# jtdingx/quadrupedal_loco

Measured on AMD Instinct MI355X. Metric: MPC QP solves/sec (Go1 SRBD N=10, 12 forces); p99 solve us, higher is better.
Workload: dtype f32

## Files before the change

### include/qloco.h

```cpp
#ifndef QLOCO_H
#define QLOCO_H

#include <stddef.h>
#include <stdint.h>

#ifdef __cplusplus
extern "C" {
#endif

#define QLOCO_ABI_VERSION 1

typedef enum qloco_status {
  QLOCO_OK = 0,
  QLOCO_MAX_ITER = 1,
  QLOCO_INFEASIBLE = 2,
  QLOCO_NAN = 3,
  QLOCO_BAD_SIZE = 4,
  QLOCO_NOT_PD = 5,
  QLOCO_DEGENERATE = 6,
  QLOCO_UB_PATH = 7,
  QLOCO_SOLVED_INACCURATE = 8,
  QLOCO_ERR_ARG = 100,
  QLOCO_ERR_DEVICE = 101,
  QLOCO_ERR_NO_GPU = 102
} qloco_status;

const char *qloco_status_string(int status);
int qloco_abi_version(void);
const char *qloco_last_error(void);

typedef struct qloco_srbd_spec {
  int32_t horizon;
  int32_t feet_per_step;
  int32_t contacts_per_step;
  int32_t output_frame;
  float dt;
  float mass;
  float inertia[9];
  float q_weights[13];
  float r_weights[12];
  float mu;
  float fz_min, fz_max;
  float rho, sigma, alpha, eps_abs, eps_rel;
  int32_t max_iter, check_termination, scaling, adaptive_rho, adaptive_rho_interval;
  float adaptive_rho_tolerance;
  int32_t warm_start;
  int32_t polish;
  int32_t literal_full_qp;
  int32_t reserved[5];
} qloco_srbd_spec;

#define QLOCO_SRBD_PERSIST_LEN(N) (100 * (N) + 4)

void qloco_srbd_spec_default(qloco_srbd_spec *spec);

int qloco_srbd_lit_tables(const qloco_srbd_spec *spec, float *gtab, int64_t gtab_len,
                          float *s_scale, float *gmx, int32_t *served);

int qloco_srbd_max_stance_vars(void);

int qloco_srbd_solve(const qloco_srbd_spec *spec, int64_t batch, const float *x0,
                     const float *x_ref, const float *feet, const uint8_t *contacts,
                     float *u0, float *u, int32_t *status, int32_t *iters, float *obj,
                     float *warm, void *stream);

int qloco_srbd_solve_ex(const qloco_srbd_spec *spec, int64_t batch, const float *x0,
                        const float *x_ref, const float *feet, const uint8_t *contacts,
                        float *u0, float *u, int32_t *status, int32_t *iters,
                        int32_t *rho_updates, float *obj, float *warm,
                        int32_t max_stance_legs, void *stream);

int64_t qloco_srbd_place_bytes(int64_t batch);
int qloco_srbd_solve_placed(const qloco_srbd_spec *spec, int64_t batch, const float *x0,
                            const float *x_ref, const float *feet, const uint8_t *contacts,
                            float *u0, float *u, int32_t *status, int32_t *iters,
                            int32_t *rho_updates, float *obj, float *warm,
                            int32_t max_stance_legs, int32_t *place, void *stream);

int qloco_srbd_place_order_host(int64_t batch, int64_t simds, int32_t check_termination,
                                const int32_t *hint, int32_t *order);

#define QLOCO_ROUTE_LIT_ONE_WAVE 1
#define QLOCO_ROUTE_LIT_TWO_WAVE 2
#define QLOCO_ROUTE_LIT_GENERIC 3
#define QLOCO_ROUTE_REDUCED 4
int qloco_srbd_route(const qloco_srbd_spec *spec);

int qloco_srbd_scratch_sets(int32_t *pinned);

int qloco_srbd_build(const qloco_srbd_spec *spec, int64_t batch, const float *x0,
                     const float *x_ref, const float *feet, const uint8_t *contacts,
                     float *H, float *g, float *lb, float *ub, float *Aqp, float *Bqp,
                     void *stream);

int qloco_gen_srbd_host(uint64_t seed, int32_t horizon, float dt, int32_t gait,
                        int64_t first, int64_t count, float *x0, float *x_ref,
                        float *feet, uint8_t *contacts);
int qloco_gen_srbd_host_strided(uint64_t seed, int32_t horizon, float dt, int32_t gait,
                                int64_t first, int64_t stride, int64_t count, float *x0,
                                float *x_ref, float *feet, uint8_t *contacts);

int qloco_eiquadprog_solve(int32_t n, int32_t p, int32_t m, int64_t batch, const double *G,
                           int64_t G_stride, const double *g0, int64_t g0_stride,
                           const double *CE, int64_t CE_stride, const double *ce0,
                           int64_t ce0_stride, const double *CI, int64_t CI_stride,
                           const double *ci0, int64_t ci0_stride, double *x, double *f,
                           int32_t *status, int32_t *iters, void *stream);
int qloco_max_gi_vars(void);
void qloco_gi_fast_limits(int32_t *n, int32_t *p, int32_t *m);
void qloco_gi_limits(int32_t *n, int32_t *p, int32_t *m);

typedef struct qloco_force_params {
  double mass;
  double alpha;
  double beta;
  double gamma;
  double fz_max;
  double mu;
} qloco_force_params;
void qloco_force_params_default(qloco_force_params *p);

int qloco_force_qp_solve(const qloco_force_params *prm, int64_t batch, const double *com_des,
                         const double *leg_des, const double *F_force_des,
                         const double *rfoot_des, const double *lfoot_des,
                         const double *base_p, const double *feet_p,
                         const double *FT_total_des, const int32_t *mode,
                         const int32_t *right_support, const double *y_coef,
                         double *F_leg_ref, double *grf_opt, double *F_leg_guess,
                         int32_t *qp_solution, int32_t *status, int32_t *iters,
                         void *stream);

int64_t qloco_force_order_ws_len(int64_t batch);
int qloco_force_qp_solve_ordered(const qloco_force_params *prm, int64_t batch,
                                 const double *com_des, const double *leg_des,
                                 const double *F_force_des, const double *rfoot_des,
                                 const double *lfoot_des, const double *base_p,
                                 const double *feet_p, const double *FT_total_des,
                                 const int32_t *mode, const int32_t *right_support,
                                 const double *y_coef, double *F_leg_ref, double *grf_opt,
                                 double *F_leg_guess, int32_t *qp_solution, int32_t *status,
                                 int32_t *iters, int32_t *order_ws, void *stream);

void qloco_force_params_hw(qloco_force_params *p);

int qloco_force_set_group_width(int gw);

int qloco_hw_torque_ff(int64_t batch, const double *Jaco, const double *grf_opt,
                       const double *grf_base, const int32_t *dynamic_count, double *tau,
                       void *stream);

int qloco_joint_torques(int64_t batch, const double *Jaco, const int32_t *swing,
                        const double *p_des, const double *p_est, const double *pv_des,
                        const double *pv_est, const double *F_leg_ref, double *tau,
                        void *stream);

#define QLOCO_BODY_STATE_LEN 32
int qloco_body_state_init_host(int64_t batch, double *state);
int qloco_body_mpc_step(int64_t batch, const int32_t *i, const double *bodyangle_state,
                        const double *zmp_ref, const double *angle_ref,
                        const double *rfoot_ref, const double *lfoot_ref,
                        const double *comacc_ref, double *state, double *com_traj,
                        int32_t *status, void *stream);
int qloco_body_indexfind(int64_t batch, const double *t, int32_t *j_period, void *stream);

int qloco_leg_fk(int64_t n, const double *q, const int32_t *leg, const double *body_p,
                 const double *body_r, double *pos, double *jac, void *stream);
int qloco_leg_ik(int64_t n, const double *pos_des, const double *q_ini, const int32_t *leg,
                 const double *body_p, const double *body_r, double *q_out, double *pos,
                 double *jac, int32_t *updates, void *stream);

#define QLOCO_GAIT_MSG_LEN 100
#define QLOCO_CTRL_MSG_LEN 25
#define QLOCO_TRAJ_MSG_LEN 100
#define QLOCO_NRT_MSG_LEN 25
#define QLOCO_RT_SCHED_LEN 8
int64_t qloco_rt_workspace_bytes(int64_t batch);
int qloco_rt_init(int64_t batch, void *workspace, void *stream);
int qloco_rt_tick(int64_t batch, void *workspace, const double *gait_msg,
                  const double *ctrl_msg, double *traj_msg, double *nrt_msg, double *gen,
                  int32_t *sched, void *stream);

int64_t qloco_servo_workspace_bytes(int64_t batch);
int qloco_servo_init(int64_t batch, void *workspace, void *stream);
int qloco_servo_force_block(const qloco_force_params *prm, int64_t batch, void *workspace,
                            const double *coma_des, const double *com_des,
                            const double *rfoot_des, const double *lfoot_des,
                            const double *body_p_des, const double *foot_des,
                            const int32_t *right_support, const int32_t *gait_mode,
                            const double *y_offset, const int32_t *loop_count,
                            const double *Jaco, const double *foot_rel_mea,
                            const double *v_est_rel, double *F_sum, double *Force_L_R,
                            double *grf_opt, double *tau, int32_t *swing,
                            int32_t *qp_solution, int32_t *status, void *stream);

#define QLOCO_NLP_STEPS 27
int qloco_support_phase(int64_t batch, const double *ts, const double *tx, const int32_t *t_int,
                        const int32_t *t_end_footstep, int32_t *bjxx, int32_t *bjx1,
                        int32_t *right_support, void *stream);

typedef struct qloco_a1_params {
  double kp_linear[3], kd_linear[3], kp_angular[3], kd_angular[3];
  double robot_mass;
  double q_diag[6];
  double r;
  double mu;
  double f_min, f_max;
  double rho, sigma, alpha, eps_abs, eps_rel, adaptive_rho_tolerance;
  int32_t max_iter, check_termination, scaling, adaptive_rho, adaptive_rho_interval;
  int32_t reserved[3];
} qloco_a1_params;
void qloco_a1_params_default(qloco_a1_params *p);
#define QLOCO_A1_STATE_LEN 54
int qloco_a1_qp_solve(const qloco_a1_params *prm, int64_t batch, const double *state,
                      const uint8_t *contacts, double *forces_body, double *qp_solution,
                      int32_t *status, int32_t *iters, int32_t *rho_updates, double *obj,
                      void *stream);

#define QLOCO_MGPU_ID_BYTES 128
enum {
  QLOCO_SHARD_CONTIGUOUS = 0,
  QLOCO_SHARD_INTERLEAVED = 1
};
typedef struct qloco_mgpu qloco_mgpu;
int qloco_mgpu_shard(int64_t total, int32_t world, int32_t rank, int32_t mode, int64_t *first,
                     int64_t *count, int64_t *stride);
int qloco_mgpu_gather_rows(int64_t total, int32_t world, int32_t mode, int64_t *rows);
int qloco_mgpu_reorder(int64_t total, int32_t world, int32_t mode, int32_t width, const float *stage,
                       float *u0_all, int32_t *status_all, int32_t *iters_all, void *stream);
int qloco_mgpu_unique_id(uint8_t *id );
int qloco_mgpu_init(qloco_mgpu **h, const uint8_t *id, int32_t world, int32_t rank, int64_t total,
                    int32_t mode);
int qloco_mgpu_info(const qloco_mgpu *h, int64_t *first, int64_t *count, int64_t *stride,
                    int64_t *padded);
// ... 223 lines not shown
```

### quadrupedal_loco_amd/_lib.py

```python
import ctypes as C
import os

HERE = os.path.dirname(os.path.abspath(__file__))
LIB_PATH = os.environ.get("QLOCO_LIB") or os.path.join(HERE, "lib", "libqloco.so")

_lib = None


class SrbdSpec(C.Structure):
    _fields_ = [
        ("horizon", C.c_int32), ("feet_per_step", C.c_int32),
        ("contacts_per_step", C.c_int32), ("output_frame", C.c_int32),
        ("dt", C.c_float), ("mass", C.c_float), ("inertia", C.c_float * 9),
        ("q_weights", C.c_float * 13), ("r_weights", C.c_float * 12),
        ("mu", C.c_float), ("fz_min", C.c_float), ("fz_max", C.c_float),
        ("rho", C.c_float), ("sigma", C.c_float), ("alpha", C.c_float),
        ("eps_abs", C.c_float), ("eps_rel", C.c_float),
        ("max_iter", C.c_int32), ("check_termination", C.c_int32), ("scaling", C.c_int32),
        ("adaptive_rho", C.c_int32), ("adaptive_rho_interval", C.c_int32),
        ("adaptive_rho_tolerance", C.c_float), ("warm_start", C.c_int32),
        ("polish", C.c_int32), ("literal_full_qp", C.c_int32), ("reserved", C.c_int32 * 5),
    ]


class ForceParams(C.Structure):
    _fields_ = [(k, C.c_double) for k in ("mass", "alpha", "beta", "gamma", "fz_max", "mu")]


class A1Params(C.Structure):
    _fields_ = [("kp_linear", C.c_double * 3), ("kd_linear", C.c_double * 3),
                ("kp_angular", C.c_double * 3), ("kd_angular", C.c_double * 3),
                ("robot_mass", C.c_double), ("q_diag", C.c_double * 6), ("r", C.c_double),
                ("mu", C.c_double), ("f_min", C.c_double), ("f_max", C.c_double),
                ("rho", C.c_double), ("sigma", C.c_double), ("alpha", C.c_double),
                ("eps_abs", C.c_double), ("eps_rel", C.c_double),
                ("adaptive_rho_tolerance", C.c_double),
                ("max_iter", C.c_int32), ("check_termination", C.c_int32),
                ("scaling", C.c_int32), ("adaptive_rho", C.c_int32),
                ("adaptive_rho_interval", C.c_int32), ("reserved", C.c_int32 * 3)]


class A1KinParams(C.Structure):
    _fields_ = [("rho_fix", (C.c_double * 5) * 4), ("rho_opt", (C.c_double * 3) * 4)]


class A1EkfParams(C.Structure):
    _fields_ = [("process_noise_pimu", C.c_double), ("process_noise_vimu", C.c_double),
                ("process_noise_pfoot", C.c_double), ("sensor_noise_pimu_rel_foot", C.c_double),
                ("sensor_noise_vimu_rel_foot", C.c_double), ("sensor_noise_zfoot", C.c_double),
                ("assume_flat_ground", C.c_int32), ("reserved", C.c_int32 * 7)]


class A1CtrlParams(C.Structure):
    _fields_ = [("counter_per_gait", C.c_double), ("counter_per_swing", C.c_double),
                ("gait_counter_speed", C.c_double * 4), ("gait_counter_reset", C.c_double * 4),
                ("default_foot_pos", C.c_double * 12), ("control_dt", C.c_double),
                ("kp_foot", C.c_double * 12), ("kd_foot", C.c_double * 12),
                ("km_foot", C.c_double * 3), ("torques_gravity", C.c_double * 12),
                ("foot_delta_x_limit", C.c_double), ("foot_delta_y_limit", C.c_double),
                ("foot_force_low", C.c_double), ("foot_swing_clearance1", C.c_double),
                ("foot_swing_clearance2", C.c_double), ("recent_contact_window", C.c_int32),
                ("terrain_window", C.c_int32), ("torque_holdoff_ticks", C.c_int32),
                ("reserved", C.c_int32 * 5)]


class NlpParams(C.Structure):
    _fields_ = [(k, C.c_double) for k in (
        "dt", "tstep", "t_min", "t_max", "footx_vmax", "footx_vmin", "footy_vmax", "footy_vmin",
        "comax_max", "comax_min", "comay_max", "comay_min", "aax", "aay", "aaxv", "aayv", "bbx", "bby",
        "rr1", "rr2", "footx_max", "footx_min", "z_c", "g", "half_hip_width", "foot_width",
        "lamda_comx", "lamda_comvx", "lamda_comy", "lamda_comvy")] + [("reserved", C.c_double * 2)]


class NlpTickParams(C.Structure):
    _fields_ = [("lift_height", C.c_double), ("hcom", C.c_double), ("reserved", C.c_double * 6)]


class NlpNodeParams(C.Structure):
    _fields_ = [(k, C.c_double) for k in ("dtx", "height_offset_time", "height_squat_time", "height_offset",
                                          "height_offsetx", "totalmass", "rad")] + [("reserved", C.c_double * 9)]


class ButterCoef(C.Structure):
    _fields_ = [(k, C.c_double) for k in ("b0", "b1", "b2", "a1", "a2", "a")]


class Go1ServoParams(C.Structure):
    _fields_ = [(k, C.c_double) for k in (
        "rt_frequency", "stand_duration", "dtx", "dt_mpc_slow", "t_period", "t_walk_start", "pi",
        "half_hip_width", "z_c")] + [("target_pos", C.c_double * 12), ("filter", ButterCoef * 15),
                                     ("force", ForceParams), ("reserved", C.c_double * 8)]


GO1_SERVO_DIAG = (("body_r_est", 3, "f8"), ("foot_rel_mea", 12, "f8"), ("v_est_rel", 12, "f8"),
                  ("Jaco_est", 36, "f8"), ("com_des", 3, "f8"), ("rfoot_des", 3, "f8"),
                  ("lfoot_des", 3, "f8"), ("coma_des", 3, "f8"), ("thetaacc_des", 3, "f8"),
                  ("comv_des", 3, "f8"), ("body_p_des", 3, "f8"), ("body_r_des", 3, "f8"),
                  ("foot_des", 12, "f8"), ("angle_des", 12, "f8"), ("Jaco", 36, "f8"),
                  ("ik_updates", 4, "i4"), ("F_sum", 6, "f8"), ("Force_L_R", 6, "f8"),
                  ("swing", 4, "i4"), ("qp_solution", 1, "i4"), ("status", 1, "i4"))


class Go1ServoDiag(C.Structure):
    _fields_ = [(k, C.c_void_p) for k, _, _ in GO1_SERVO_DIAG]


vp = C.c_void_p
i64 = C.c_int64
i32 = C.c_int32

SIGNATURES = {
    "qloco_status_string": (C.c_char_p, [C.c_int]),
    "qloco_abi_version": (C.c_int, []),
    "qloco_last_error": (C.c_char_p, []),
    "qloco_srbd_spec_default": (None, [C.POINTER(SrbdSpec)]),
    "qloco_srbd_max_stance_vars": (C.c_int, []),
    "qloco_srbd_route": (C.c_int, [C.POINTER(SrbdSpec)]),
    "qloco_srbd_lit_tables": (C.c_int, [C.POINTER(SrbdSpec), vp, i64, vp, vp, vp]),
    "qloco_srbd_solve": (C.c_int, [C.POINTER(SrbdSpec), i64, vp, vp, vp, vp, vp, vp, vp, vp,
                                   vp, vp, vp]),
    "qloco_srbd_solve_ex": (C.c_int, [C.POINTER(SrbdSpec), i64, vp, vp, vp, vp, vp, vp, vp, vp,
                                      vp, vp, vp, i32, vp]),
    "qloco_srbd_solve_placed": (C.c_int, [C.POINTER(SrbdSpec), i64, vp, vp, vp, vp, vp, vp, vp, vp,
                                          vp, vp, vp, i32, vp, vp]),
    "qloco_srbd_place_bytes": (i64, [i64]),
    "qloco_srbd_place_order_host": (C.c_int, [i64, i64, i32, vp, vp]),
    "qloco_srbd_build": (C.c_int, [C.POINTER(SrbdSpec), i64, vp, vp, vp, vp, vp, vp, vp, vp,
                                   vp, vp, vp]),
    "qloco_gen_srbd_host": (C.c_int, [C.c_uint64, i32, C.c_float, i32, i64, i64, vp, vp, vp,
                                      vp]),
    "qloco_gen_srbd_host_strided": (C.c_int, [C.c_uint64, i32, C.c_float, i32, i64, i64, i64, vp,
                                              vp, vp, vp]),
    "qloco_eiquadprog_solve": (C.c_int, [i32, i32, i32, i64, vp, i64, vp, i64, vp, i64, vp, i64,
                                         vp, i64, vp, i64, vp, vp, vp, vp, vp]),
    "qloco_max_gi_vars": (C.c_int, []),
    "qloco_gi_limits": (None, [C.c_void_p, C.c_void_p, C.c_void_p]),
    "qloco_gi_fast_limits": (None, [C.c_void_p, C.c_void_p, C.c_void_p]),
    "qloco_srbd_scratch_sets": (C.c_int, [C.c_void_p]),
    "qloco_force_params_default": (None, [C.POINTER(ForceParams)]),
    "qloco_force_qp_solve": (C.c_int, [C.POINTER(ForceParams), i64] + [vp] * 18),
    "qloco_force_qp_solve_ordered": (C.c_int, [C.POINTER(ForceParams), i64] + [vp] * 19),
    "qloco_force_order_ws_len": (i64, [i64]),
    "qloco_leg_fk": (C.c_int, [i64] + [vp] * 7),
    "qloco_leg_ik": (C.c_int, [i64] + [vp] * 10),
    "qloco_joint_torques": (C.c_int, [i64] + [vp] * 9),
    "qloco_force_params_hw": (None, [C.POINTER(ForceParams)]),
    "qloco_force_set_group_width": (C.c_int, [C.c_int]),
    "qloco_hw_torque_ff": (C.c_int, [i64] + [vp] * 6),
    "qloco_body_state_init_host": (C.c_int, [i64, vp]),
    "qloco_body_mpc_step": (C.c_int, [i64] + [vp] * 10),
    "qloco_body_indexfind": (C.c_int, [i64, vp, vp, vp]),
    "qloco_rt_workspace_bytes": (C.c_int64, [i64]),
    "qloco_rt_init": (C.c_int, [i64, vp, vp]),
    "qloco_rt_tick": (C.c_int, [i64, vp, vp, vp, vp, vp, vp, vp, vp]),
    "qloco_servo_workspace_bytes": (C.c_int64, [i64]),
    "qloco_servo_init": (C.c_int, [i64, vp, vp]),
    "qloco_servo_force_block": (C.c_int, [C.POINTER(ForceParams), i64] + [vp] * 22),
    "qloco_support_phase": (C.c_int, [i64] + [vp] * 8),
    "qloco_a1_params_default": (None, [C.POINTER(A1Params)]),
    "qloco_a1_qp_solve": (C.c_int, [C.POINTER(A1Params), i64] + [vp] * 9),
    "qloco_a1_kin_params_default": (None, [C.POINTER(A1KinParams)]),
    "qloco_a1_leg_kin": (C.c_int, [C.POINTER(A1KinParams), i64] + [vp] * 16),
    "qloco_a1_ekf_params_default": (None, [C.POINTER(A1EkfParams)]),
    "qloco_a1_ekf_workspace_bytes": (C.c_int64, [i64]),
    "qloco_a1_ekf_init": (C.c_int, [C.POINTER(A1EkfParams), i64, vp, vp, vp, vp]),
    "qloco_a1_ekf_update": (C.c_int, [C.POINTER(A1EkfParams), i64] + [vp] * 13),
    "qloco_a1_ekf_get_state": (C.c_int, [i64, vp, vp, vp, vp]),
    "qloco_a1_ekf_set_state": (C.c_int, [i64, vp, vp, vp, vp]),
    "qloco_a1_ctrl_params_default": (None, [C.POINTER(A1CtrlParams)]),
    "qloco_a1_ctrl_workspace_bytes": (C.c_int64, [i64]),
    "qloco_a1_ctrl_reset": (C.c_int, [C.POINTER(A1CtrlParams), i64, vp, vp]),
    "qloco_a1_ctrl_plan_swing": (C.c_int, [C.POINTER(A1CtrlParams), i64] + [vp] * 21),
    "qloco_a1_ctrl_terrain": (C.c_int, [C.POINTER(A1CtrlParams), i64] + [vp] * 6),
    "qloco_a1_ctrl_joint_torques": (C.c_int, [C.POINTER(A1CtrlParams), i64] + [vp] * 5),
    "qloco_a1_ctrl_get_state": (C.c_int, [i64, vp, vp, vp]),
    "qloco_a1_ctrl_set_state": (C.c_int, [i64, vp, vp, vp]),
    "qloco_nlp_params_default": (None, [C.POINTER(NlpParams)]),
    "qloco_nlp_workspace_bytes": (C.c_int64, [i64]),
    "qloco_nlp_init": (C.c_int, [C.POINTER(NlpParams), i64] + [vp] * 5),
    "qloco_nlp_step_timing": (C.c_int, [C.POINTER(NlpParams), i64] + [vp] * 13),
    "qloco_nlp_get_state": (C.c_int, [i64, vp, vp, vp]),
    "qloco_nlp_set_state": (C.c_int, [i64, vp, vp, vp]),
    "qloco_nlp_set_group_width": (C.c_int, [C.c_int]),
    "qloco_nlp_tick_params_default": (None, [C.POINTER(NlpTickParams)]),
    "qloco_nlp_tick_workspace_bytes": (C.c_int64, [i64]),
    "qloco_nlp_tick_init": (C.c_int, [C.POINTER(NlpParams), C.POINTER(NlpTickParams), i64] + [vp] * 6),
    "qloco_nlp_tick": (C.c_int, [C.POINTER(NlpParams), C.POINTER(NlpTickParams), i64] + [vp] * 18),
    "qloco_nlp_tick_set_group_width": (C.c_int, [C.c_int]),
    "qloco_nlp_tick_get_state": (C.c_int, [i64, vp, vp, vp]),
    "qloco_nlp_tick_set_state": (C.c_int, [i64, vp, vp, vp]),
    "qloco_nlp_node_params_default": (None, [C.POINTER(NlpNodeParams)]),
    "qloco_nlp_node_workspace_bytes": (C.c_int64, [i64]),
    "qloco_nlp_node_init": (C.c_int, [C.POINTER(NlpParams), C.POINTER(NlpTickParams), C.POINTER(NlpNodeParams),
                                      i64] + [vp] * 7),
    "qloco_nlp_node_tick": (C.c_int, [C.POINTER(NlpParams), C.POINTER(NlpTickParams), C.POINTER(NlpNodeParams),
                                      i64] + [vp] * 8),
    "qloco_nlp_node_set_form": (C.c_int, [C.c_int]),
    "qloco_nlp_node_get_state": (C.c_int, [i64, vp, vp, vp]),
    "qloco_nlp_node_set_state": (C.c_int, [i64, vp, vp, vp]),
    "qloco_go1_servo_params_default": (None, [C.POINTER(Go1ServoParams)]),
    "qloco_go1_servo_workspace_bytes": (C.c_int64, [i64]),
    "qloco_go1_servo_init": (C.c_int, [C.POINTER(Go1ServoParams), i64, vp, vp]),
    "qloco_go1_servo_tick": (C.c_int, [C.POINTER(Go1ServoParams), i64, vp, i64] + [vp] * 9 +
                             [C.POINTER(Go1ServoDiag), vp, vp]),
    "qloco_go1_servo_get_state": (C.c_int, [i64, vp, vp, vp]),
    "qloco_go1_servo_set_state": (C.c_int, [i64, vp, vp, vp]),
    "qloco_mgpu_shard": (C.c_int, [i64, i32, i32, i32, vp, vp, vp]),
    "qloco_mgpu_gather_rows": (C.c_int, [i64, i32, i32, vp]),
    "qloco_mgpu_reorder": (C.c_int, [i64, i32, i32, i32, vp, vp, vp, vp, vp]),
    "qloco_mgpu_unique_id": (C.c_int, [vp]),
    "qloco_mgpu_init": (C.c_int, [vp, vp, i32, i32, i64, i32]),
    "qloco_mgpu_info": (C.c_int, [vp, vp, vp, vp, vp]),
    "qloco_mgpu_solve": (C.c_int, [vp, C.POINTER(SrbdSpec), vp, vp, vp, vp, vp, vp, vp, vp, i32, vp]),
    "qloco_mgpu_destroy": (C.c_int, [vp]),
}


class QlocoError(RuntimeError):
    pass


def lib():
    global _lib
    if _lib is None:
        if not os.path.exists(LIB_PATH):
            raise QlocoError(
                "libqloco.so not built (%s); run `python -m quadrupedal_loco_amd.build` "
                "or __graft_entry__.build()" % LIB_PATH)
        L = C.CDLL(LIB_PATH, mode=C.RTLD_GLOBAL)
        for name, (res, args) in SIGNATURES.items():
            if not hasattr(L, name):
                continue
            f = getattr(L, name)
            f.restype = res
            f.argtypes = args
        _lib = L
    return _lib


def missing_symbols():
    L = lib()
    return [n for n in SIGNATURES if not hasattr(L, n)]


def check(status, what):
    if status != 0:
        L = lib()
        msg = L.qloco_status_string(status).decode()
        err = L.qloco_last_error().decode()
        raise QlocoError("%s failed: %s %s" % (what, msg, err))


def ptr(t):
    if t is None:
        return None
    if hasattr(t, "data_ptr"):
        return C.c_void_p(t.data_ptr())
    return C.c_void_p(t.ctypes.data)
```

### quadrupedal_loco_amd/csrc/qloco_srbd_core.hpp

```cpp
#pragma once
#include <stddef.h>
#include <stdint.h>

#include <type_traits>

#include "qloco_common.hpp"
#include "qloco_dpp.inc"
#include "qloco_srbd_spec.hpp"

namespace qloco {

struct SrbdArgs {
  int N, feet_per_step, contacts_per_step, output_frame;
  float dt, mass;
  float inertia[9];
  float q2[13];
  float r2[12];
  float mu, fz_min, fz_max;
  float rho, sigma, alpha, eps_abs, eps_rel;
  int max_iter, check_termination, scaling, adaptive_rho, rho_interval;
  float rho_tol;
  int warm_start;
  int literal;
  int leg_lo, leg_hi;
  int64_t batch;
  const float *x0, *xref, *feet;
  const uint8_t *contacts;
  float *u0, *u, *obj, *warm;
  int *status, *iters, *rho_updates;
  const int *list;
  const int *count;
  int *hint;
  const int *order;
  int lit_tables;
  float lit_sq;
  float lit_gmx;
  alignas(16) float lit_gtab[kLitN * kLitN * 6];
};

inline void srbd_args_from_spec(const qloco_srbd_spec *spec, SrbdArgs *a) {
  a->N = spec->horizon;
  a->feet_per_step = spec->feet_per_step;
  a->contacts_per_step = spec->contacts_per_step;
  a->output_frame = spec->output_frame;
  a->dt = spec->dt;
  a->mass = spec->mass;
  for (int k = 0; k < 9; ++k) a->inertia[k] = spec->inertia[k];
  srbd_doubled_weights(spec, a->q2, a->r2);
  a->mu = spec->mu;
  a->fz_min = spec->fz_min;
  a->fz_max = spec->fz_max;
  a->rho = spec->rho;
  a->sigma = spec->sigma;
  a->alpha = spec->alpha;
  a->eps_abs = spec->eps_abs;
  a->eps_rel = spec->eps_rel;
  a->max_iter = spec->max_iter;
  a->check_termination = spec->check_termination;
  a->scaling = spec->scaling;
  a->adaptive_rho = spec->adaptive_rho;
  a->rho_interval = spec->adaptive_rho_interval;
  a->rho_tol = spec->adaptive_rho_tolerance;
  a->warm_start = spec->warm_start;
  a->literal = spec->literal_full_qp ? 1 : 0;
}

typedef float f2v __attribute__((ext_vector_type(2)));
typedef float f4v __attribute__((ext_vector_type(4)));

template <int W>
struct Row {
  float k[64 * W];
};
#define KE(K, c) ((K).k[(c)])

template <int CTRL>
__device__ __forceinline__ float dpp(float v) {
  return __builtin_bit_cast(float, __builtin_amdgcn_mov_dpp(__builtin_bit_cast(int, v), CTRL, 0xF,
                                                            0xF, false));
}
template <int C, int E>
struct ColLoop {
  template <class F>
  static __device__ __forceinline__ void run(F &&f) {
    f(std::integral_constant<int, C>{});
    ColLoop<C + 1, E>::run(f);
  }
};
template <int E>
struct ColLoop<E, E> {
  template <class F>
  static __device__ __forceinline__ void run(F &&) {}
};
template <int C>
__device__ __forceinline__ float dpp_col(const f4v &d) {
  constexpr int e = C & 3;
  const float v = e == 0 ? d.x : (e == 1 ? d.y : (e == 2 ? d.z : d.w));
  return dpp<0x150 + (C >> 2)>(v);
}

__device__ __forceinline__ int opaque_tid() {
  int t = threadIdx.x;
  asm volatile("" : "+v"(t));
  return t;
}

__device__ __forceinline__ int fresh_lane() {
  int l;
  asm volatile("v_mbcnt_lo_u32_b32 %0, -1, 0\n\tv_mbcnt_hi_u32_b32 %0, -1, %0" : "=v"(l));
  return l;
}

__device__ __forceinline__ float sgpr_f(float v) {
  return __builtin_bit_cast(float, __builtin_amdgcn_readfirstlane(__builtin_bit_cast(int, v)));
}

__device__ __forceinline__ float lane_prev(float v) { return dpp<0x138>(v); }
__device__ __forceinline__ float lane_next(float v) { return dpp<0x130>(v); }
__device__ __forceinline__ float rlane(float v, int l) {
  return __builtin_bit_cast(float, __builtin_amdgcn_readlane(__builtin_bit_cast(int, v), l));
}

__device__ __forceinline__ float wmax(float v) {
  v = fmaxf(v, dpp<0xB1>(v));
  v = fmaxf(v, dpp<0x4E>(v));
  v = fmaxf(v, dpp<0x124>(v));
  v = fmaxf(v, dpp<0x128>(v));
  return fmaxf(fmaxf(rlane(v, 0), rlane(v, 16)), fmaxf(rlane(v, 32), rlane(v, 48)));
}
__device__ __forceinline__ float wsum(float v) {
  v += dpp<0xB1>(v);
  v += dpp<0x4E>(v);
  v += dpp<0x124>(v);
  v += dpp<0x128>(v);
  return (rlane(v, 0) + rlane(v, 16)) + (rlane(v, 32) + rlane(v, 48));
}

#define QL_DMAXU(U, CTRL)                                                       \
  asm("s_nop 1\n\tv_max_u32_dpp %0, %0, %0 " CTRL " bank_mask:0xf" : "+v"(U))
__device__ __forceinline__ float wmax_nonneg(float v) {
  unsigned u = __builtin_bit_cast(unsigned, v);
  QL_DMAXU(u, "quad_perm:[1,0,3,2] row_mask:0xf");
  QL_DMAXU(u, "quad_perm:[2,3,0,1] row_mask:0xf");
  QL_DMAXU(u, "row_ror:4 row_mask:0xf");
  QL_DMAXU(u, "row_ror:8 row_mask:0xf");
  QL_DMAXU(u, "row_bcast:15 row_mask:0xa");
  QL_DMAXU(u, "row_bcast:31 row_mask:0xc");
  return __builtin_bit_cast(float, __builtin_amdgcn_readlane(u, 63));
}

#define QL_DMAXU6(CTRL)                                      \
  "v_max_u32_dpp %0, %0, %0 " CTRL " bank_mask:0xf\n\t"      \
  "v_max_u32_dpp %1, %1, %1 " CTRL " bank_mask:0xf\n\t"      \
  "v_max_u32_dpp %2, %2, %2 " CTRL " bank_mask:0xf\n\t"      \
  "v_max_u32_dpp %3, %3, %3 " CTRL " bank_mask:0xf\n\t"      \
  "v_max_u32_dpp %4, %4, %4 " CTRL " bank_mask:0xf\n\t"      \
  "v_max_u32_dpp %5, %5, %5 " CTRL " bank_mask:0xf\n\t"
__device__ __forceinline__ void wmax_nonneg6(float (&v)[6]) {
  unsigned u[6];
#pragma unroll
  for (int k = 0; k < 6; ++k) u[k] = __builtin_bit_cast(unsigned, v[k]);
  asm("s_nop 1\n\t"
      QL_DMAXU6("quad_perm:[1,0,3,2] row_mask:0xf")
      QL_DMAXU6("quad_perm:[2,3,0,1] row_mask:0xf")
      QL_DMAXU6("row_ror:4 row_mask:0xf")
      QL_DMAXU6("row_ror:8 row_mask:0xf")
      QL_DMAXU6("row_bcast:15 row_mask:0xa")
      QL_DMAXU6("row_bcast:31 row_mask:0xc")
      : "+v"(u[0]), "+v"(u[1]), "+v"(u[2]), "+v"(u[3]), "+v"(u[4]), "+v"(u[5]));
#pragma unroll
  for (int k = 0; k < 6; ++k) v[k] = __builtin_bit_cast(float, __builtin_amdgcn_readlane(u[k], 63));
}

__device__ __forceinline__ void k0k2(float ja, float jb, float Nf, float &K0, float &K2) {
  const float M = fmaxf(ja, jb);
  const float T = Nf - M;
  const float al = M - ja, be = M - jb;
  const float S1 = 0.5f * T * (T - 1.0f);
  const float S2 = rintf(S1 * (2.0f * T - 1.0f) * (1.0f / 3.0f));
  K0 = T;
  K2 = S2 + (al + be) * S1 + al * be * T;
}

constexpr float kGjExactPivot = 16.0f;

static_assert(sizeof(SrbdArgs) <= 4096, "kernel argument segment");
// ... 8 lines not shown
```

### quadrupedal_loco_amd/csrc/qloco_srbd_lit.hip

```cpp
#include <math.h>
#include <stddef.h>

#include <type_traits>

#include "qloco_srbd_core.hpp"
#include "qloco_srbd_model.hpp"
#include "qloco_srbd_place.hpp"

namespace qloco {

constexpr int kLitWpe = 4;
constexpr int kLit2Wpe = 2;

template <int W>
struct LitLds {
  static constexpr int NS = W == 1 ? kLitN : kLitN2;
  static constexpr int NT = NS;
  float Bb[6][12];
  float Te[6][6];
  float q2[16], r2[12], x0[16];
  float ctf[4 * NT];
  float pad0[W == 1 ? 0 : 24];
  f4v bc[W][W][16];
  float av[W][2][64];
// ... 1175 lines not shown
          }
#pragma unroll
          for (int h = 0; h < 2; ++h)
            zn[h] = {__builtin_amdgcn_fmed3f(vv[h].x, zlw[h], zhi[h]), __builtin_amdgcn_fmed3f(vv[h].y, -INFINITY, 0.0f)};
#pragma unroll
          for (int h = 0; h < 2; ++h) {
            const f2v rv = {rva[h][0], rva[h][1]};
            y[h] = __builtin_elementwise_fma(rv, zr[h] - zn[h], y[h]);
            z[h] = zn[h];
          }
        }
      }
      iter = ui(iter);
      S.sc[wv].iter = iter;
      const bool fin = iter >= a.max_iter;
      const bool can_check = ctm && iter > 0 && (iter % ctm == 0);
      const bool do_rho = interval && iter > 0 && (iter % interval == 0);
      if (!(can_check || do_rho || fin)) continue;
      float o[6], r[6];
      residuals(o, r, do_rho);
      const float cinv = uf(S.sc[wv].cinv), qn0 = uf(S.sc[wv].qn0);
      const float pri_res = o[0], dua_res = cinv * o[3];
      if (can_check) {
        const float eps_p = a.eps_abs + a.eps_rel * fmaxf(o[1], o[2]);
        const float eps_d = a.eps_abs + a.eps_rel * cinv * fmaxf(fmaxf(qn0, o[4]), o[5]);
        if (pri_res < eps_p && dua_res < eps_d) {
          S.sc[wv].status = QLOCO_OK;
          break;
        }
      }
      if (do_rho) {
        const float pn = r[0] / (fmaxf(r[1], r[2]) + 1e-30f);
        const float dn = r[3] / (fmaxf(fmaxf(uf(S.sc[wv].qn1), r[4]), r[5]) + 1e-30f);
        const float rho = uf(S.sc[wv].rho);
        float rho_new = rho * sqrtf(pn / (dn + 1e-30f));
        rho_new = fminf(fmaxf(rho_new, 1e-6f), 1e6f);
        if (rho_new > rho * a.rho_tol || rho_new < rho / a.rho_tol) {
          const int nup = ui(S.sc[wv].rho_updates) + 1;
          S.sc[wv].rho = sgpr_f(rho_new);
          S.sc[wv].rho_updates = nup;
          if (!fin) {
            refactor = true;
            break;
          }
        }
      }
      if (fin) {
        float e_abs = a.eps_abs, e_rel = a.eps_rel;
        asm volatile("" : "+v"(e_abs), "+v"(e_rel));
        const float ep = 10.f * e_abs + 10.f * e_rel * fmaxf(o[1], o[2]);
        const float ed = 10.f * e_abs + 10.f * e_rel * cinv * fmaxf(fmaxf(qn0, o[4]), o[5]);
        S.sc[wv].status = __builtin_amdgcn_readfirstlane((pri_res < ep && dua_res < ed) ? QLOCO_SOLVED_INACCURATE
                                                                                          : QLOCO_MAX_ITER);
        break;
      }
    }
    if (!refactor) break;
  }

  const int lane_o = fresh_lane();
  const int tid_o = W == 1 ? lane_o : (int)threadIdx.x;
  float xu[2];
#pragma unroll
  for (int h = 0; h < 2; ++h) xu[h] = valid[h] ? x[h] * S.dr[wv][h][lane_o] : 0.0f;
  float px[2];
  p_times_x(px);
  const float cinv = uf(S.sc[wv].cinv);
  int status = ui(S.sc[wv].status);
  float ob = 0.0f;
#pragma unroll
  for (int h = 0; h < 2; ++h) ob += valid[h] ? cinv * (0.5f * x[h] * px[h] + S.qvl[wv][h][lane_o] * x[h]) : 0.0f;
  const float objp = bsum<W>(S, wsum(ob), wv);
  const bool bad = !isfinite(objp);
  if (bad) status = QLOCO_NAN;
  if (a.u) {
    float *uo = a.u + b * 12 * N + 12 * so;
#pragma unroll
    for (int h = 0; h < 2; ++h)
      if (valid[h]) uo[60 * h + lane_o] = bad ? NAN : xu[h];
  }
  {
    const float n1 = lane_next(xu[0]), n2 = lane_next(n1);
    const float p1 = lane_prev(xu[0]), p2 = lane_prev(p1);
    const float f0 = comp == 0 ? xu[0] : (comp == 1 ? p1 : p2);
    const float f1 = comp == 0 ? n1 : (comp == 1 ? xu[0] : p1);
    const float f2 = comp == 0 ? n2 : (comp == 1 ? n1 : xu[0]);
    if (tid_o < 12) {
      float o = xu[0];
      if (a.output_frame == 1) {
        const float yw = S.x0[2], cw = cosf(yw), sw = sinf(yw);
        o = comp == 0 ? (cw * f0 - sw * f1) : (comp == 1 ? (sw * f0 + cw * f1) : f2);
      }
      a.u0[b * 12 + lane_o] = bad ? NAN : o;
    }
  }
  if (prec) {
    QL_LIT_LANE_INDICES(lxo);
    for (int k = tid_o; k < NP + 4; k += 64 * W)
      if (k < 84 * N || k >= 96 * N) prec[k] = 0.0f;
    __syncthreads();
#pragma unroll
    for (int h = 0; h < 2; ++h) {
      if (!valid[h]) continue;
      const int vidx = 12 * step[h] + 3 * leg[h] + comp, rbase = 20 * step[h] + 5 * leg[h] + 2 * comp;
      prec[vidx] = x[h];
      prec[52 * N + vidx] = xu[h];
      prec[12 * N + rbase] = z[h].x;
      prec[32 * N + rbase] = y[h].x;
      const f2v e = row_e(h);
      prec[64 * N + rbase] = cinv * e.x * y[h].x;
      if (xy) {
        prec[12 * N + rbase + 1] = z[h].y;
        prec[32 * N + rbase + 1] = y[h].y;
        prec[64 * N + rbase + 1] = cinv * e.y * y[h].y;
      }
    }
    for (int k = tid_o; k < 4 * N; k += 64 * W) prec[96 * N + k] = S.ctf[k];
    if (tid_o == 0) {
      prec[NP] = S.sc[wv].rho;
      prec[NP + 1] = 1.0f;
    }
  }
  if (WS && a.warm_start == 1) {
    QL_LIT_LANE_INDICES(lxo);
    const int nu = 12 * N, ncn = 20 * N;
    float *wx = a.warm + b * (nu + ncn);
    float *wy = wx + nu;
    for (int k = tid_o; k < nu + ncn; k += 64 * W) wx[k] = 0.0f;
    __syncthreads();
#pragma unroll
    for (int h = 0; h < 2; ++h) {
      if (!valid[h]) continue;
      wx[12 * step[h] + 3 * leg[h] + comp] = xu[h];
      const int rbase = 20 * step[h] + 5 * leg[h] + 2 * comp;
      const f2v e = row_e(h);
      wy[rbase] = cinv * e.x * y[h].x;
      if (xy) wy[rbase + 1] = cinv * e.y * y[h].y;
    }
  }
  if (tid_o == 0) {
    if (a.status) a.status[b] = status;
    if (a.iters) a.iters[b] = S.sc[wv].iter;
    if (a.hint) a.hint[b] = S.sc[wv].iter;
    if (a.rho_updates) a.rho_updates[b] = S.sc[wv].rho_updates;
    if (a.obj) a.obj[b] = objp;
  }
}

template <bool WS>
__global__ __launch_bounds__(64) __attribute__((amdgpu_waves_per_eu(kLitWpe)))
void srbd_lit_kernel(const SrbdArgs a) {
  __shared__ __attribute__((aligned(16))) LitLds<1> S;
  int64_t i = blockIdx.x;
  if (a.order && a.hint[-kPlaceHeader] == a.batch) i = a.order[blockIdx.x];
  if (i < 0 || i >= a.batch) return;
  srbd_lit_one<1, WS>(a, S, i);
}

template <bool WS>
__global__ __launch_bounds__(128) __attribute__((amdgpu_waves_per_eu(kLit2Wpe)))
void srbd_lit2_kernel(const SrbdArgs a) {
  __shared__ __attribute__((aligned(16))) LitLds<2> S;
  const int64_t i = blockIdx.x;
  if (i >= a.batch) return;
  srbd_lit_one<2, WS>(a, S, i);
}

static int device_simds(int *simds) {
  constexpr int kDevs = 64;
  static int cached[kDevs];
  int dev = 0, cus = 0;
  QLOCO_HIP_CHECK(hipGetDevice(&dev), "hipGetDevice");
  if (dev >= 0 && dev < kDevs && cached[dev] > 0) {
    *simds = cached[dev];
    return QLOCO_OK;
  }
  QLOCO_HIP_CHECK(hipDeviceGetAttribute(&cus, hipDeviceAttributeMultiprocessorCount, dev),
                  "hipDeviceGetAttribute");
  *simds = 4 * cus;
  if (dev >= 0 && dev < kDevs) cached[dev] = *simds;
  return QLOCO_OK;
}

int srbd_lit_launch(const SrbdArgs &a, bool warm, int32_t *place, int simds, hipStream_t stream) {
  const dim3 grid((unsigned)a.batch);
  if (a.N < 1 || a.N > kLitN2) return QLOCO_BAD_SIZE;
  if (a.N <= kLitN) {
    if (warm) {
      hipLaunchKernelGGL(srbd_lit_kernel<true>, grid, dim3(64), 0, stream, a);
    } else {
      SrbdArgs ap = a;
      bool placed = false;
      if (place) {
        if (simds <= 0) {
          const int rc = device_simds(&simds);
          if (rc != QLOCO_OK) return rc;
        }
        placed = a.batch > simds && a.batch <= (int64_t)kLitWpe * simds;
      }
      if (placed) {
        ap.hint = place + kPlaceHeader;
        ap.order = place + kPlaceHeader + a.batch;
      }
      hipLaunchKernelGGL(srbd_lit_kernel<false>, grid, dim3(64), 0, stream, ap);
      QLOCO_HIP_CHECK(hipGetLastError(), "srbd_lit_kernel launch");
      if (placed) return srbd_place_launch(place, a.batch, simds, a.check_termination, stream);
    }
    QLOCO_HIP_CHECK(hipGetLastError(), "srbd_lit_kernel launch");
  } else {
    if (warm)
      hipLaunchKernelGGL(srbd_lit2_kernel<true>, grid, dim3(128), 0, stream, a);
    else
      hipLaunchKernelGGL(srbd_lit2_kernel<false>, grid, dim3(128), 0, stream, a);
    QLOCO_HIP_CHECK(hipGetLastError(), "srbd_lit2_kernel launch");
  }
  return QLOCO_OK;
}

}
```

### quadrupedal_loco_amd/csrc/qloco_srbd_place.hip

```cpp
#include <vector>

#include "qloco_common.hpp"
#include "qloco_srbd_core.hpp"
#include "qloco_srbd_place.hpp"

namespace qloco {

constexpr int kPlaceThreads = 1024;

__global__ __launch_bounds__(kPlaceThreads) void srbd_place_kernel(int *place, int batch, int simds,
                                                                    int check_termination) {
  __shared__ int count[kPlaceClasses];
  __shared__ int cursor[kPlaceClasses];
  const int t = threadIdx.x;
  const int *hint = place + kPlaceHeader;
  int *order = place + kPlaceHeader + batch;
  if (t < kPlaceClasses) count[t] = 0;
  __syncthreads();
  for (int i = t; i < batch; i += kPlaceThreads)
    atomicAdd(&count[place_class(hint[i], check_termination)], 1);
  __syncthreads();
  if (t < kPlaceClasses) {
    int first = 0;
    for (int c = t + 1; c < kPlaceClasses; ++c) first += count[c];
    cursor[t] = first;
  }
  __syncthreads();
  for (int i = t; i < batch; i += kPlaceThreads) {
    const int rank = atomicAdd(&cursor[place_class(hint[i], check_termination)], 1);
    order[place_position(rank, batch, simds)] = i;
  }
  __syncthreads();
  if (t == 0) place[0] = batch;
}

int srbd_place_launch(int32_t *place, int64_t batch, int simds, int check_termination,
                      hipStream_t stream) {
  hipLaunchKernelGGL(srbd_place_kernel, dim3(1), dim3(kPlaceThreads), 0, stream, place, (int)batch,
                     simds, check_termination);
  QLOCO_HIP_CHECK(hipGetLastError(), "srbd_place_kernel launch");
  return QLOCO_OK;
}

}

extern "C" int64_t qloco_srbd_place_bytes(int64_t batch) {
  if (batch < 0 || batch > (int64_t)1 << 30) return 0;
  return (int64_t)sizeof(int32_t) * (qloco::kPlaceHeader + 2 * batch);
}

extern "C" int qloco_srbd_place_order_host(int64_t batch, int64_t simds, int32_t check_termination,
                                           const int32_t *hint, int32_t *order) {
  using namespace qloco;
  if (!hint || !order || simds < 1 || batch <= simds || batch > 4 * simds ||
      batch > (int64_t)1 << 30)
    return QLOCO_ERR_ARG;
  std::vector<int64_t> cursor(kPlaceClasses + 1, 0);
  for (int64_t i = 0; i < batch; ++i) ++cursor[place_class(hint[i], check_termination)];
  int64_t first = 0;
  for (int c = kPlaceClasses - 1; c >= 0; --c) {
    const int64_t n = cursor[c];
    cursor[c] = first;
    first += n;
  }
  for (int64_t i = 0; i < batch; ++i) {
    const int64_t rank = cursor[place_class(hint[i], check_termination)]++;
    order[place_position(rank, batch, simds)] = (int32_t)i;
  }
  return QLOCO_OK;
}
```

### quadrupedal_loco_amd/csrc/qloco_srbd_place.hpp

```cpp
#pragma once
#include <stdint.h>

#include "qloco_common.hpp"

namespace qloco {

constexpr int kPlaceHeader = 4;
constexpr int kPlaceClasses = 256;

__host__ __device__ inline int place_class(int hint, int check_termination) {
  const int c = hint / (check_termination > 1 ? check_termination : 1);
  return c < 0 ? 0 : (c > kPlaceClasses - 1 ? kPlaceClasses - 1 : c);
}

__host__ __device__ inline int64_t place_rank(int64_t p, int64_t B, int64_t S) {
  const int64_t s = p % S, q = p / S;
  if (q == 0) return s;
  const int64_t T = B - S, m = (T + S - 1) / S, r = T - (m - 1) * S;
  return B - 1 - (s * (m - 1) + (s < r ? s : r) + (q - 1));
}

__host__ __device__ inline int64_t place_position(int64_t k, int64_t B, int64_t S) {
  if (k < S) return k;
  const int64_t T = B - S, m = (T + S - 1) / S, r = T - (m - 1) * S;
  const int64_t j = B - 1 - k;
  int64_t s, c;
  if (j < r * m) {
    s = j / m;
    c = j - s * m;
  } else {
    const int64_t jj = j - r * m;
    s = r + jj / (m - 1);
    c = jj - (s - r) * (m - 1);
  }
  return s + S * (c + 1);
}

}
```

Before: 11.49 million.

## Remap placed block order with tiered per-SIMD assignment in lit kernel

The lit kernel no longer reads the placement order directly by block index. It now maps the block index through a new place_assign function that splits SIMDs into three tiers, so the second-round slots get the cheapest remaining problems and the longest tail solves are spread differently across SIMDs. This targets load imbalance and tail latency when batch exceeds the number of SIMDs. It adds per-block integer arithmetic and depends on assumptions about how the hardware dispatches blocks to SIMDs. A host helper is also added to expose the mapping for testing.

```diff
diff --git a/include/qloco.h b/include/qloco.h
--- a/include/qloco.h
+++ b/include/qloco.h
@@ -79,6 +79,8 @@
 
 int qloco_srbd_place_order_host(int64_t batch, int64_t simds, int32_t check_termination,
                                 const int32_t *hint, int32_t *order);
+
+int qloco_srbd_place_assign_host(int64_t batch, int64_t simds, int32_t *rank_of_position);
 
 #define QLOCO_ROUTE_LIT_ONE_WAVE 1
 #define QLOCO_ROUTE_LIT_TWO_WAVE 2
diff --git a/quadrupedal_loco_amd/_lib.py b/quadrupedal_loco_amd/_lib.py
--- a/quadrupedal_loco_amd/_lib.py
+++ b/quadrupedal_loco_amd/_lib.py
@@ -125,6 +125,7 @@
                                           vp, vp, vp, i32, vp, vp]),
     "qloco_srbd_place_bytes": (i64, [i64]),
     "qloco_srbd_place_order_host": (C.c_int, [i64, i64, i32, vp, vp]),
+    "qloco_srbd_place_assign_host": (C.c_int, [i64, i64, vp]),
     "qloco_srbd_build": (C.c_int, [C.POINTER(SrbdSpec), i64, vp, vp, vp, vp, vp, vp, vp, vp,
                                    vp, vp, vp]),
     "qloco_gen_srbd_host": (C.c_int, [C.c_uint64, i32, C.c_float, i32, i64, i64, vp, vp, vp,
diff --git a/quadrupedal_loco_amd/csrc/qloco_srbd_core.hpp b/quadrupedal_loco_amd/csrc/qloco_srbd_core.hpp
--- a/quadrupedal_loco_amd/csrc/qloco_srbd_core.hpp
+++ b/quadrupedal_loco_amd/csrc/qloco_srbd_core.hpp
@@ -32,6 +32,7 @@
   const int *count;
   int *hint;
   const int *order;
+  int place_simds;
   int lit_tables;
   float lit_sq;
   float lit_gmx;
diff --git a/quadrupedal_loco_amd/csrc/qloco_srbd_lit.hip b/quadrupedal_loco_amd/csrc/qloco_srbd_lit.hip
--- a/quadrupedal_loco_amd/csrc/qloco_srbd_lit.hip
+++ b/quadrupedal_loco_amd/csrc/qloco_srbd_lit.hip
@@ -1351,7 +1351,11 @@
 void srbd_lit_kernel(const SrbdArgs a) {
   __shared__ __attribute__((aligned(16))) LitLds<1> S;
   int64_t i = blockIdx.x;
-  if (a.order && a.hint[-kPlaceHeader] == a.batch) i = a.order[blockIdx.x];
+  if (a.order && a.hint[-kPlaceHeader] == a.batch) {
+    const int64_t at = place_position(place_assign(i, a.batch, a.place_simds), a.batch, a.place_simds);
+    if (at < 0 || at >= a.batch) return;
+    i = a.order[at];
+  }
   if (i < 0 || i >= a.batch) return;
   srbd_lit_one<1, WS>(a, S, i);
 }
@@ -1400,6 +1404,7 @@
       if (placed) {
         ap.hint = place + kPlaceHeader;
         ap.order = place + kPlaceHeader + a.batch;
+        ap.place_simds = simds;
       }
       hipLaunchKernelGGL(srbd_lit_kernel<false>, grid, dim3(64), 0, stream, ap);
       QLOCO_HIP_CHECK(hipGetLastError(), "srbd_lit_kernel launch");
diff --git a/quadrupedal_loco_amd/csrc/qloco_srbd_place.hip b/quadrupedal_loco_amd/csrc/qloco_srbd_place.hip
--- a/quadrupedal_loco_amd/csrc/qloco_srbd_place.hip
+++ b/quadrupedal_loco_amd/csrc/qloco_srbd_place.hip
@@ -69,3 +69,13 @@
   }
   return QLOCO_OK;
 }
+
+extern "C" int qloco_srbd_place_assign_host(int64_t batch, int64_t simds,
+                                            int32_t *rank_of_position) {
+  using namespace qloco;
+  if (!rank_of_position || simds < 1 || batch <= simds || batch > 4 * simds ||
+      batch > (int64_t)1 << 30)
+    return QLOCO_ERR_ARG;
+  for (int64_t p = 0; p < batch; ++p) rank_of_position[p] = (int32_t)place_assign(p, batch, simds);
+  return QLOCO_OK;
+}
diff --git a/quadrupedal_loco_amd/csrc/qloco_srbd_place.hpp b/quadrupedal_loco_amd/csrc/qloco_srbd_place.hpp
--- a/quadrupedal_loco_amd/csrc/qloco_srbd_place.hpp
+++ b/quadrupedal_loco_amd/csrc/qloco_srbd_place.hpp
@@ -36,4 +36,24 @@
   return s + S * (c + 1);
 }
 
+__host__ __device__ inline int64_t place_assign(int64_t p, int64_t B, int64_t S) {
+  const int64_t s = p % S, q = p / S;
+  if (q == 0) return s;
+  const int64_t T = B - S, m = (T + S - 1) / S, r = T - (m - 1) * S;
+  const int64_t A1 = m < 2 ? S : S / 64, A2 = A1 > 3 * S / 16 ? A1 : 3 * S / 16;
+  const int64_t n2 = A2 - A1, n3 = S - A2;
+  const int64_t before = s * (m - 1) + (s < r ? s : r);
+  if (s < A1) return B - 1 - (before + (q - 1));
+  if (s < A2) {
+    if (q == 1) return S + n3 + (A2 - 1 - s);
+    return B - 1 - (before - (s - A1) + (q - 2));
+  }
+  const int64_t i = s - A2;
+  if (q == 1) return S + (n3 - 1 - i);
+  const int64_t taken = A2 * (m - 1) + (A2 < r ? A2 : r) - n2;
+  if (q == m) return B - 1 - (taken + i);
+  const int64_t last = r - A2 < 0 ? 0 : (r - A2 > n3 ? n3 : r - A2);
+  return B - 1 - (taken + last + (m - 1 - q) * n3 + i);
 }
+
+}
```

After: 12.12 million, median of 6. 5.5% higher.
